# CITlabRostock/citlab-article-separation-new

Hardware: AMD Instinct MI355X
Metric: newspaper pages/sec (ARU-Net seg + GNN relation) at 3000x4500 px (higher is better)
Workload: dtype f32s

## Files before the change

citlab-article-separation-new_amd/csrc/aru_engine.hip:

```cpp
#include <algorithm>
#include <cmath>
#include <cstdlib>
#include <memory>

#include "aru_kernels.h"
#include "res8_kernels.h"
#include "res8v_kernels.h"
#include "bf16_kernels.h"
#include "res8w_kernels.h"
#include "res8ws_kernels.h"
#include "level0_plan.h"
#include "launch_plan.h"
#include "convr_kernels.h"
#include "split_kernels.h"
#include "pyr_kernels.h"
#include "asep_common.h"
#include "aru_pack.h"

using namespace asep;

namespace {

struct Tensor {
    float* p = nullptr;
// ... 26 lines not shown
    asep_aru_cfg cfg{};
    std::map<std::string, PackedConv> convs;
    struct ResB { int C = 0; bf16_t* d_w = nullptr; float* d_b = nullptr; };
    std::map<std::string, ResB> resb;
    std::map<std::string, float*> taps;
    bf16_t* d_r8b_down_w = nullptr;
    float* d_r8b_down_b = nullptr;
    bf16_t* d_r8b_up_w1 = nullptr;
    bf16_t* d_r8f_up_w1 = nullptr;
    bf16_t* d_r8f_down_w1 = nullptr;
    float* d_r8b_down_w1r = nullptr;
    bool use_res32 = true;
    int walk_mode = 1;
    bool use_deconvs = true;
    bool use_convr = true;
    unsigned char* d_zero_trash = nullptr;
    int fused_act = 0;
    bool use_walk = true;
    bf16_t* d_r8b_up_w = nullptr;
    float* d_r8b_up_b = nullptr;
    float* d_r8b_up_b1 = nullptr;
    DirectConv det_first, att_first;
    float* d_r8_down_wr = nullptr;
    float* d_r8_down_br = nullptr;
    float* d_r8_up_w1 = nullptr;
    float* d_r8_up_wr = nullptr;
    float* d_r8_up_br = nullptr;
    float* d_r8_up_b1 = nullptr;
    float* d_r8v_down_wr = nullptr;
    float* d_r8v_up_w1 = nullptr;
    float* d_r8v_up_wr = nullptr;
    bool r8_valu = true;
    bool use_split_walk = true;
    bf16_t* d_r8ws_down_w = nullptr;
    bf16_t* d_r8ws_up_w = nullptr;
    bf16_t* d_r8ws_up_w1 = nullptr;
    bool use_fused8 = true;
    bool fused8_wanted = true;
    bool fused8_var = false;
    float* d_att_head = nullptr;
    bf16_t* d_att_headb = nullptr;
    float* d_logit_w = nullptr;
    float* d_logit_b = nullptr;
    float* d_logit_wd = nullptr;
    float* d_stats = nullptr;
    const float* const* page_stats = nullptr;
    double* d_sums = nullptr;
    struct Lane {
        hipStream_t s = nullptr;
        bool own_stream = false;
        hipStream_t side = nullptr;
        hipEvent_t ev_fork = nullptr, ev_join = nullptr, ev_begin = nullptr, ev_done = nullptr;
        hipStream_t bside = nullptr;
        hipEvent_t ev_bfork = nullptr, ev_bjoin = nullptr;
        BufferPool pool;
        ~Lane() {
            if (ev_fork) (void)hipEventDestroy(ev_fork);
            if (ev_bfork) (void)hipEventDestroy(ev_bfork);
            if (ev_bjoin) (void)hipEventDestroy(ev_bjoin);
            if (ev_join) (void)hipEventDestroy(ev_join);
            if (ev_begin) (void)hipEventDestroy(ev_begin);
            if (ev_done) (void)hipEventDestroy(ev_done);
            if (side) (void)hipStreamDestroy(side);
            if (bside) (void)hipStreamDestroy(bside);
            if (own_stream && s) (void)hipStreamDestroy(s);
        }
// ... 471 lines not shown
    TL out;
    for (const Tensor& t : in) {
        if (kind == POOL_CHANSUM) out.push_back(new_tensor(m, t.H, t.W, 1));
        else out.push_back(new_tensor(m, cdiv(t.H, 2), cdiv(t.W, 2), t.C));
    }
    stream_pass<PoolArgs>(m, in, kind == POOL_MAX ? "maxpool2_kernel" : (kind == POOL_AVG_C1 ? "avgpool2_c1_kernel" : (kind == POOL_AVG_C3 ? "avgpool2_cn_kernel<3>" : "chansum_kernel")), POOL_ITEMS,
        [&](PoolProb& p, size_t i, Chunk& k) {
            k.bytes += tbytes(in[i]) + tbytes(out[i]);
            p.in = in[i].p; p.out = out[i].p; p.H = in[i].H; p.W = in[i].W; p.Ho = out[i].H; p.Wo = out[i].W;
            return kind == POOL_MAX ? out[i].count() / 4 : (size_t)out[i].H * out[i].W;
        }, [&](const PoolArgs& a, dim3 grid) {
            if (kind == POOL_MAX) hipLaunchKernelGGL(maxpool2_kernel, grid, dim3(256), 0, m->stream, a);
            else if (kind == POOL_AVG_C1) hipLaunchKernelGGL(avgpool2_c1_kernel, grid, dim3(256), 0, m->stream, a);
            else if (kind == POOL_AVG_C3) launch_avgpool_c3(m, a, grid);
            else hipLaunchKernelGGL(chansum_kernel, grid, dim3(256), 0, m->stream, a);
        });
    return out;
}

int grid_1d(size_t n) { return (int)std::min<size_t>((n + 255) / 256, 256 * 8); }

std::string res8_what(bool up, const TL& l) {
    return (up ? "unet_up_0 (conv1[16->8]+3xconvR+add) " : "unet_down_0 (conv1+3xconvR+add+pool) ") + dims_of(l);
}

bool r8v_fits(const TL& l) {
    for (const Tensor& t : l)
        if ((size_t)t.H * t.W >= ((size_t)1 << 28)) return false;
    return true;
}

bool r8ws_fits(const Tensor& t) { return walk_region(t.H, t.W).fits; }
bool r8ws_on(asep_aru* m) { return m->split && m->use_split_walk && m->r8_valu && m->cfg.activation == 0 && m->d_r8ws_down_w; }
const int32_t* r8ws_frame_units(asep_aru* m, const Res8Args& a, const std::vector<bool>& walk, int* count) {
    std::string key = "f";
    for (int i = 0; i < a.nprob; ++i) key += ":" + std::to_string(a.p[i].H) + "x" + std::to_string(a.p[i].W) + (walk[i] ? "w" : "t");
    std::vector<int32_t> units;
    for (int i = 0; i < a.nprob; ++i) frame_units(a.p[i].H, a.p[i].W, a.p[i].tiles_x, a.p[i].tile_begin, walk[i], R8_OW, R8_OH * R8_NP, &units);
    *count = (int)units.size();
    auto it = m->sched_cache.find(key);
    if (it != m->sched_cache.end()) return it->second;
    if (units.empty()) return nullptr;
    const int32_t* d = put_table(m, units);
    if (d) m->sched_cache[key] = d;
    return d;
}

void run_res8ws(asep_aru* m, bool up, const Res8Args& a, const std::vector<bool>& walk, const std::string& what) {
    Res8WSArgs wa{};
    int n = 0, items = 0;
    double flops = 0, bytes = 0;
    long strip_rows = 0;
    for (int i = 0; i < a.nprob; ++i) {
        if (!walk[i]) continue;
        const Res8Prob& q = a.p[i];
        Res8WSProb& p = wa.p[n++];
        if (up) { p.skip = q.img; p.dec = q.in1; }
        else { p.img = q.img; p.stats = q.stats; p.pool = q.pool; }
        p.out = q.out;
        p.H = q.H; p.W = q.W;
        const WalkRegion r = walk_region(p.H, p.W);
        p.n_strips = r.n_strips;
        p.y_end = r.y_end;
        strip_rows += (long)r.n_strips * r.rows();
        flops += 2.0 * r.pixels() * (9.0 * (up ? 16 : 1) * 8 + 3 * 9.0 * 64);
        bytes += r.pixels() * ((up ? 64.0 : 4.0) + 32.0 + (p.pool ? 8.0 : 0.0));
    }
    if (!n) return;
    const int band = walk_band(strip_rows, m->num_cus, 4);
    for (int i = 0; i < n; ++i) {
        Res8WSProb& p = wa.p[i];
        p.band = band;
// ... 22 lines not shown
}

void run_res8(asep_aru* m, bool up, const TL& in0, const TL* in1, const std::vector<const float*>& stats, bool want_pool, TL* d_out, TL* pool_out) {
    for (const Tensor& t : in0) {
        d_out->push_back(new_tensor(m, t.H, t.W, 8));
        if (want_pool) pool_out->push_back(new_tensor(m, cdiv(t.H, 2), cdiv(t.W, 2), 8));
    }
    const size_t lds = up ? R8_UP_LDS : R8_DOWN_LDS;
    const char* layer = up ? "unet_up_0" : "unet_down_0";
    for_chunks<Res8Args>(in0.size(), 0.0, [&](Res8Prob& p, size_t i, Chunk& k) {
        k.bytes += tbytes(in0[i]) + (up ? tbytes((*in1)[i]) : 0.0) + tbytes((*d_out)[i]) + (want_pool ? tbytes((*pool_out)[i]) : 0.0);
        p.img = in0[i].p; p.in1 = up ? (*in1)[i].p : nullptr; p.stats = stats.empty() ? nullptr : stats[i];
        p.out = (*d_out)[i].p; p.pool = want_pool ? (*pool_out)[i].p : nullptr;
        p.H = in0[i].H; p.W = in0[i].W;
        set_tiles(p, k.units.next_tiles(p.H, p.W, R8_OW, R8_OH * R8_NP));
        k.flops += 2.0 * in0[i].H * in0[i].W * (9.0 * (up ? 16 : 1) * 8 + 3 * 9.0 * 64);
    }, [&](Res8Args& a, const Chunk& c) {
        const int tiles = c.units.total;
        const double flops = c.flops, bytes = c.bytes;
        const TL sub = c.sub(in0);
        const bool valu = m->r8_valu && r8v_fits(sub);
        if (up) { a.w1 = valu ? m->d_r8v_up_w1 : m->d_r8_up_w1; a.b1 = m->d_r8_up_b1; }
        else { a.w1 = m->det_first.d_w; a.b1 = m->det_first.d_b; }
        a.wr = (const f32x4*)(up ? (valu ? m->d_r8v_up_wr : m->d_r8_up_wr) : (valu ? m->d_r8v_down_wr : m->d_r8_down_wr));
        a.br = up ? m->d_r8_up_br : m->d_r8_down_br;
        const int actv = m->cfg.activation;
        const Res8Kernel k = res8_kernel(up, valu, actv);
        a.sched = tile_schedule(m, a, std::min(tiles, m->num_cus), R8_OH * R8_NP);
        if (valu && r8ws_on(m) && (!up || m->d_r8ws_up_w1)) {
            std::vector<bool> walk(a.nprob);
            bool any = false;
            for (int i = 0; i < a.nprob; ++i) { walk[i] = r8ws_fits(sub[i]); any = any || walk[i]; }
            if (any) {
                int nu = 0;
                Res8Args f = a;
                f.sched = r8ws_frame_units(m, a, walk, &nu);
                if (!f.sched) { set_error("level-0 frame schedule: device allocation failed"); throw ArgError(); }
                f.total_tiles = nu;
                {
                    const double share = (double)nu / tiles;
                    ProfScope ps(m, k.name, flops * share, std::string(layer) + " frame " + dims_of(sub));
                    ps.bytes = bytes * share;
                    hipLaunchKernelGGL(k.fn, dim3(std::min(nu, m->num_cus)), dim3(R8_THREADS), lds, m->stream, f);
                }
                run_res8ws(m, up, a, walk, res8_what(up, sub));
                return;
            }
        }
        ProfScope ps(m, k.name, flops, res8_what(up, sub));
        ps.bytes = bytes;
        if (actv && !valu) { set_error("level-0 block of an elu / leaky graph: image too large for the vector-ALU kernel"); throw ArgError(); }
        hipLaunchKernelGGL(k.fn, dim3(std::min(tiles, m->num_cus)), dim3(R8_THREADS), lds, m->stream, a);
    });
}

void run_res8b_tiles(asep_aru* m, bool up, const TL& a0, const TL* a1, const std::vector<const float*>& stats, bool want_pool, const TL& outs, const TL* pool_out);

void run_res8w(asep_aru* m, bool up, const TL& in0, const TL* dec, const std::vector<const float*>& stats, const TL& outs, const TL* pools) {
    for (size_t c = 0; c < num_chunks(in0.size()); ++c) {
        const size_t b0 = chunk_begin(c), b1 = chunk_end(in0.size(), c);
        Res8WArgs wa{};
        Res8WBArgs ba{};
        double flops = 0, bytes = 0, wshare = 0;
        long strip_rows = 0;
        for (size_t i = b0; i < b1; ++i) {
            Res8WProb& p = wa.p[i - b0];
            if (up) { p.skip = in0[i].bp(); p.dec = (*dec)[i].bp(); }
            else { p.img = in0[i].p; p.stats = stats.empty() ? nullptr : stats[i]; p.pool = pools ? (*pools)[i].bp() : nullptr; }
            p.out = outs[i].bp();
            p.H = in0[i].H; p.W = in0[i].W;
            const WalkRegion r = walk_region(p.H, p.W);
            p.n_strips = r.n_strips;
            p.y_end = r.y_end;
            strip_rows += (long)r.n_strips * r.rows();
            bytes += tbytes(in0[i]) + (up ? tbytes((*dec)[i]) : 0.0) + tbytes(outs[i]) + (pools ? tbytes((*pools)[i]) : 0.0);
            flops += 2.0 * p.H * p.W * (9.0 * (up ? 16 : 1) * 8 + 3 * 9.0 * 64);
            wshare += r.pixels();
        }
// ... 952 lines not shown
    }
    if (cfg->input_pyramid && cfg->compute_dtype == 1) {
        set_error("asep_aru_load: the input-pyramid graph (RU_v2) is served by the fp32 engines (compute_dtype 0 or 2): the bf16 engine's fused block "
                  "tails round conv1's result to bfloat16 before the pooled page's term could be added");
        return nullptr;
    }
    std::map<std::string, HostTensor> blob;
    if (!parse_blob(weight_blob, nbytes, blob)) return nullptr;
    std::map<std::string, std::vector<float>> taps;
    if (cfg->input_pyramid) {
        try {
            blob = split_pyramid_blob(blob, *cfg, taps);
        } catch (const PackRefusal&) {
            return nullptr;
        }
    }
    warn_ignored_switches();
    std::unique_ptr<asep_aru> m(new asep_aru());
    m->cfg = *cfg;
    m->bf16 = cfg->compute_dtype == 1;
    m->split = cfg->compute_dtype == 2;
    if (const char* e = getenv("ASEP_FUSE_POOL")) m->fuse_pool = atoi(e) != 0;
    if (const char* e = getenv("ASEP_FUSE_ACT")) m->fuse_act = atoi(e) != 0;
    if (const char* e = getenv("ASEP_C12")) m->use_c12 = atoi(e) != 0;
    if (const char* e = getenv("ASEP_FUSED8")) m->use_fused8 = atoi(e) != 0;
    m->fused8_wanted = m->use_fused8;
    if (variant) m->use_fused8 = false;
    if (const char* e = getenv("ASEP_R8_VALU")) m->r8_valu = atoi(e) != 0;
    m->fused8_var = variant && !cfg->plain_u && cfg->activation != 0 && m->fused8_wanted && m->r8_valu && m->fuse_act && !m->bf16;
    if (const char* e = getenv("ASEP_XCD_SCHED")) m->use_xcd_sched = atoi(e) != 0;
    if (const char* e = getenv("ASEP_BF_RES32")) m->use_res32 = atoi(e) != 0;
    if (const char* e = getenv("ASEP_BF_CONVR")) m->use_convr = atoi(e) != 0;
    if (const char* e = getenv("ASEP_SPLIT_DECONV")) m->use_deconvs = atoi(e) != 0;
    if (const char* e = getenv("ASEP_SPLIT_WALK")) m->use_split_walk = atoi(e) != 0;
    if (const char* e = getenv("ASEP_BF_WALK")) { m->walk_mode = atoi(e); m->use_walk = m->walk_mode != 0; }
    if (const char* e = getenv("ASEP_LANES")) { m->num_lanes = std::max(1, std::min(4, atoi(e))); m->lanes_forced = true; }
    for (int l = 0; l < m->num_lanes; ++l) {
        std::unique_ptr<asep_aru::Lane> L(new asep_aru::Lane());
        bool ok = hipStreamCreateWithFlags(&L->side, hipStreamNonBlocking) == hipSuccess &&
                  hipStreamCreateWithFlags(&L->bside, hipStreamNonBlocking) == hipSuccess &&
                  hipEventCreateWithFlags(&L->ev_fork, hipEventDisableTiming) == hipSuccess &&
                  hipEventCreateWithFlags(&L->ev_bfork, hipEventDisableTiming) == hipSuccess &&
                  hipEventCreateWithFlags(&L->ev_bjoin, hipEventDisableTiming) == hipSuccess &&
                  hipEventCreateWithFlags(&L->ev_join, hipEventDisableTiming) == hipSuccess &&
                  hipEventCreateWithFlags(&L->ev_begin, hipEventDisableTiming) == hipSuccess &&
                  hipEventCreateWithFlags(&L->ev_done, hipEventDisableTiming) == hipSuccess;
        if (ok && l > 0) { ok = hipStreamCreateWithFlags(&L->s, hipStreamNonBlocking) == hipSuccess; L->own_stream = ok; }
        if (!ok) { set_error("asep_aru_load: cannot create streams/events for lane %d", l); return nullptr; }
        m->lanes.push_back(std::move(L));
    }
    m->cur = m->lanes[0].get();
    for (const auto& t : taps) m->taps[t.first] = m->put(t.second);
    try {
        load_weights(m.get(), blob, variant);
    } catch (const PackRefusal&) {
        return nullptr;
    }
    {
        hipDeviceProp_t prop;
        int dev = 0;
        if (hipGetDevice(&dev) == hipSuccess && hipGetDeviceProperties(&prop, dev) == hipSuccess && prop.multiProcessorCount > 0)
            m->num_cus = prop.multiProcessorCount;
    }
    m->d_stats = m->alloc<float>(2);
    m->d_sums = m->alloc<double>(2);
    m->d_zero_trash = m->alloc<unsigned char>(8192);
    ASEP_HIP_CHECK_THROW(hipMemset(m->d_zero_trash, 0, 8192));
// ... 230 lines not shown
```

citlab-article-separation-new_amd/csrc/level0_plan.h:

```cpp
#pragma once
#include <algorithm>
#include <cstddef>
#include <cstdint>
#include <vector>

namespace asep {

constexpr int R8W_TW = 24;
constexpr int R8W_X0 = 32, R8W_Y0 = 16;

struct WalkRegion {
    int n_strips;
    int y_end;
    int xr;
    bool fits;
    int rows() const { return y_end - R8W_Y0; }
    double pixels() const { return (double)n_strips * R8W_TW * rows(); }
    int bands(int band) const { return (rows() + band - 1) / band; }
    int items(int band) const { return n_strips * bands(band); }
};
inline WalkRegion walk_region(int H, int W) {
    WalkRegion r;
    r.n_strips = (W - 4 - R8W_X0) / R8W_TW;
    r.y_end = R8W_Y0 + 2 * ((H - 4 - R8W_Y0) / 2);
    r.xr = R8W_X0 + R8W_TW * r.n_strips;
    r.fits = r.n_strips >= 4 && H - 4 - R8W_Y0 >= 32 && (size_t)H * W < ((size_t)1 << 28);
    return r;
}

inline int walk_band(long strip_rows, int num_cus, int waves_per_cu) {
    const long slots = (long)waves_per_cu * num_cus;
    const int band = (int)std::min<long>(256, std::max<long>(32, strip_rows / (6 * slots)));
    return (band + 1) & ~1;
}

inline void frame_units(int H, int W, int tiles_x, int tile_begin, bool walk, int unit_w, int unit_h, std::vector<int32_t>* units) {
    const WalkRegion r = walk_region(H, W);
    const int tiles_y = (H + unit_h - 1) / unit_h;
    for (int y = 0; y < tiles_y; ++y)
        for (int x = 0; x < tiles_x; ++x) {
            const int ux0 = x * unit_w, ux1 = std::min(ux0 + unit_w, W), uy0 = y * unit_h, uy1 = std::min(uy0 + unit_h, H);
            const bool frame = !walk || ux0 < R8W_X0 || ux1 > r.xr || uy0 < R8W_Y0 || uy1 > r.y_end;
            if (frame) units->push_back(tile_begin + y * tiles_x + x);
        }
}

struct BorderRect { int x0, y0, x1, y1; };
struct BorderPlan {
    int H, W;
    int nbx;
    int nby;
    int y_end, xr;
    int tiles() const { return 2 * nbx + 2 * nby; }
    BorderRect rect(int t) const {
        int x0, y0, ymax, xmax;
        if (t < nbx) { x0 = 32 * t; y0 = 0; ymax = R8W_Y0; xmax = W; }
        else if (t < 2 * nbx) { x0 = 32 * (t - nbx); y0 = y_end; ymax = H; xmax = W; }
        else if (t < 2 * nbx + nby) { x0 = 0; y0 = R8W_Y0 + 16 * (t - 2 * nbx); ymax = y_end; xmax = R8W_X0; }
        else { x0 = xr; y0 = R8W_Y0 + 16 * (t - 2 * nbx - nby); ymax = y_end; xmax = W; }
        return {x0, y0, std::min(x0 + 32, xmax), std::min(y0 + 16, ymax)};
    }
};
inline BorderPlan border_plan(int H, int W) {
    const WalkRegion r = walk_region(H, W);
    return {H, W, (W + 31) / 32, (r.rows() + 15) / 16, r.y_end, r.xr};
}

}
```

citlab-article-separation-new_amd/csrc/res8_kernels.h:

```cpp
#pragma once
#include "aru_kernels.h"

namespace asep {

#ifdef ASEP_R8_TIMELINE
__device__ unsigned long long r8_tl[16][8][64];
__device__ unsigned long long r8_clk[4];
#define R8_MARK() do { if (blockIdx.x < 16 && lane == 0 && tl_n < 64) r8_tl[blockIdx.x][wave][tl_n++] = clock64(); } while (0)
#else
#define R8_MARK() do { } while (0)
#endif

constexpr int R8_OH = 16, R8_OW = 58;
constexpr int R8_FH = R8_OH + 8;
constexpr int R8_PITCH = 72;
constexpr int R8_IMGP = 76;
constexpr int R8_WAVES = 8;
constexpr int R8_THREADS = R8_WAVES * 64;
#ifndef R8_NP_VALUE
#define R8_NP_VALUE 4
#endif
constexpr int R8_NP = R8_NP_VALUE;

struct Res8Prob {
    const float* img;
    const float* in1;
    const float* stats;
    float* out;
    float* pool;
    int H, W;
    int tiles_x, tile_begin;
};
struct Res8Args {
    Res8Prob p[MAXP];
    int nprob, total_tiles;
    const float* w1;
    const float* b1;
    const f32x4* wr;
    const float* br;
    const int32_t* sched;
};

__device__ __forceinline__ int res8_tile_of(const Res8Args& a, int k) { return a.sched ? a.sched[k] : k; }

__device__ __forceinline__ f32x4 relu4i(f32x4 v) {
    typedef int i32x4 __attribute__((ext_vector_type(4)));
    i32x4 i = __builtin_bit_cast(i32x4, v);
    i.x = max(i.x, 0); i.y = max(i.y, 0); i.z = max(i.z, 0); i.w = max(i.w, 0);
    return __builtin_bit_cast(f32x4, i);
}

__device__ __forceinline__ void r8_load_w(const f32x4* __restrict__ base, int lane, f32x4 (&A)[6]) {
    typedef const f32x4 __attribute__((address_space(1)))* gptr;
    gptr q = (gptr)(base + lane);
    asm volatile("" : "+v"(q));
#pragma unroll
    for (int c = 0; c < 6; ++c) A[c] = q[c * 64];
}

__device__ __forceinline__ int r8_px(int x, int hf) {
#ifdef R8_NO_SWIZZLE
    return x * 8 + hf * 4;
#else
    return ((x >> 1) << 4) + (((((x & 1) << 1) | hf) ^ ((x >> 2) & 3)) << 2);
// ... 440 lines not shown
```

citlab-article-separation-new_amd/csrc/res8v_kernels.h:

```cpp
#pragma once
#include "res8_kernels.h"

namespace asep {

typedef float f32x2 __attribute__((ext_vector_type(2)));
typedef const float __attribute__((address_space(4)))* r8v_cptr;
typedef char __attribute__((address_space(3)))* r8v_lds;

#ifndef R8V_WINO
#define R8V_WINO 0
#endif
#ifndef R8V_WINO_GS
#define R8V_WINO_GS 16
#endif
constexpr int R8V_FILTER = R8V_WINO ? 768 : 576;


__device__ __forceinline__ int r8v_px(int x, int hf) {
    const int P = x >> 1;
    const int g = ((P >> 2) & 1) | ((((P >> 1) ^ (P >> 3)) & 1) << 1);
    return (P << 4) + (((((x & 1) << 1) | hf) ^ g) << 2);
}

template <int ACT>
__device__ __forceinline__ f32x4 r8v_act(f32x4 v) {
    if constexpr (ACT == 0) return relu4i(v);
    else return act4(v, ACT);
}
__device__ __forceinline__ f32x4 r8v_ld(r8v_lds p) { return *reinterpret_cast<const f32x4 __attribute__((address_space(3)))*>(p); }
__device__ __forceinline__ void r8v_st(r8v_lds p, f32x4 v) { *reinterpret_cast<f32x4 __attribute__((address_space(3)))*>(p) = v; }

template <int ODD>
__device__ __forceinline__ void r8v_fma(f32x2& acc, f32x2 pair, f32x2 w) {
    if (ODD) asm("v_pk_fma_f32 %0, %1, %2, %0 op_sel:[1,0,0]" : "+v"(acc) : "v"(pair), "s"(w));
// ... 124 lines not shown
}

template <bool RELU_IN, int ACT = 0>
__device__ __forceinline__ void r8v_conv(const r8v_lds (&a)[4][2], r8v_cptr wl, f32x2 (&acc0)[4], f32x2 (&acc1)[4]) {
    if constexpr (R8V_WINO) r8v_conv_wino<RELU_IN, ACT>(a, wl, acc0, acc1);
    else r8v_conv_direct<RELU_IN, ACT>(a, wl, acc0, acc1);
}

__device__ __forceinline__ f32x4 r8v_lo(const f32x2 (&a)[4]) { return f32x4{a[0].x, a[0].y, a[1].x, a[1].y}; }
__device__ __forceinline__ f32x4 r8v_hi(const f32x2 (&a)[4]) { return f32x4{a[2].x, a[2].y, a[3].x, a[3].y}; }
__device__ __forceinline__ f32x4 r8v_max4(f32x4 a, f32x4 b) { return f32x4{fmaxf(a.x, b.x), fmaxf(a.y, b.y), fmaxf(a.z, b.z), fmaxf(a.w, b.w)}; }
__device__ __forceinline__ f32x4 r8v_upper4(f32x4 v) {
    return f32x4{from_upper_half(v.x), from_upper_half(v.y), from_upper_half(v.z), from_upper_half(v.w)};
}

__device__ __forceinline__ void r8v_pixel_offsets(int tid, int (&poff)[7][2]) {
#pragma unroll
    for (int j = 0; j < 7; ++j) { poff[j][0] = r8v_px(2 * (tid & 31) + j, 0) * 4; poff[j][1] = r8v_px(2 * (tid & 31) + j, 1) * 4; }
}
__device__ __forceinline__ void r8v_window(r8v_lds (&a)[4][2], float* sm, const int (&poff)[7][2], int j0, int row_bytes) {
    asm volatile("" : "+v"(row_bytes));
#pragma unroll
    for (int i = 0; i < 4; ++i)
#pragma unroll
        for (int hf = 0; hf < 2; ++hf) { a[i][hf] = (r8v_lds)reinterpret_cast<char*>(sm) + (poff[j0 + i][hf] + row_bytes); asm volatile("" : "+v"(a[i][hf])); }
}


template <bool RELU_IN, bool FINAL, bool POOL, int ACT = 0>
__device__ __forceinline__ void res8v_stage(float* __restrict__ sm, const float* __restrict__ IN, int in_r0, float* __restrict__ OUT, int out_r0,
                                            int row_start, int nrows, int out_c0, const float* __restrict__ w,
                                            const float* __restrict__ bias, int tid, const int (&poff)[7][2], bool interior,
                                            int fy0, int fx0, int H, int W,
                                            const float* __restrict__ T, int t_r0, float* __restrict__ gout, float* __restrict__ gpool) {
    const int x = out_c0 + 2 * (tid & 31);
    const int gx = fx0 + x;
    const int d_out = FINAL ? 0 : (int)(OUT - IN) * 4 + (in_r0 + 1 - out_r0) * R8_PITCH * 32;
    const int d_t = FINAL ? (int)(T - IN) * 4 + (in_r0 + 1 - t_r0) * R8_PITCH * 32 : 0;
#pragma unroll 1
    for (int r = tid >> 5; r < nrows; r += 16) {
        r8v_cptr wl = (r8v_cptr)w, bl = (r8v_cptr)bias;
        asm volatile("" : "+s"(wl));
        f32x2 acc0[4], acc1[4];
#pragma unroll
        for (int q = 0; q < 4; ++q) { acc0[q] = f32x2{bl[2 * q], bl[2 * q + 1]}; acc1[q] = acc0[q]; }
        const int row = row_start + r;
        r8v_lds a[4][2];
        r8v_window(a, sm, poff, out_c0 - 1, ((int)(IN - sm) + (row - 1 - in_r0) * R8_PITCH * 8) * 4);
        r8v_conv<RELU_IN, ACT>(a, wl, acc0, acc1);
        const int gy = fy0 + row;
        f32x4 p0l = r8v_lo(acc0), p0h = r8v_hi(acc0), p1l = r8v_lo(acc1), p1h = r8v_hi(acc1);
        if (!FINAL) {
            p0l = r8v_act<ACT>(p0l); p0h = r8v_act<ACT>(p0h); p1l = r8v_act<ACT>(p1l); p1h = r8v_act<ACT>(p1h);
            if (!interior) {
                const bool oky = gy >= 0 && gy < H;
                const bool ok0 = oky && gx >= 0 && gx < W, ok1 = oky && gx + 1 >= 0 && gx + 1 < W;
                const f32x4 z = f32x4{0.f, 0.f, 0.f, 0.f};
                p0l = ok0 ? p0l : z; p0h = ok0 ? p0h : z; p1l = ok1 ? p1l : z; p1h = ok1 ? p1h : z;
            }
            r8v_st(a[1][0] + d_out, p0l);
            r8v_st(a[1][1] + d_out, p0h);
            r8v_st(a[2][0] + d_out, p1l);
            r8v_st(a[2][1] + d_out, p1h);
        } else {
            p0l = r8v_act<ACT>(p0l + r8v_ld(a[1][0] + d_t));
            p0h = r8v_act<ACT>(p0h + r8v_ld(a[1][1] + d_t));
            p1l = r8v_act<ACT>(p1l + r8v_ld(a[2][0] + d_t));
            p1h = r8v_act<ACT>(p1h + r8v_ld(a[2][1] + d_t));
            const bool oky = interior || gy < H;
            const bool ok0 = x >= 4 && x < 4 + R8_OW && (interior || gx < W), ok1 = x + 1 >= 4 && x + 1 < 4 + R8_OW && (interior || gx + 1 < W);
            float* o = gout + ((unsigned)gy * (unsigned)W + (unsigned)gx) * 8u;
            if (ok0 && oky) { *reinterpret_cast<f32x4*>(o) = p0l; *reinterpret_cast<f32x4*>(o + 4) = p0h; }
            if (ok1 && oky) { *reinterpret_cast<f32x4*>(o + 8) = p1l; *reinterpret_cast<f32x4*>(o + 12) = p1h; }
            if (POOL && gpool) {
                f32x4 ml = ok1 ? r8v_max4(p0l, p1l) : p0l, mh = ok1 ? r8v_max4(p0h, p1h) : p0h;
                const f32x4 ul = r8v_upper4(ml), uh = r8v_upper4(mh);
                if ((tid & 32) == 0 && ok0 && oky) {
                    if (interior || gy + 1 < H) { ml = r8v_max4(ml, ul); mh = r8v_max4(mh, uh); }
                    const unsigned Wp = (unsigned)(W + 1) >> 1;
                    float* po = gpool + ((unsigned)(gy >> 1) * Wp + (unsigned)(gx >> 1)) * 8u;
                    *reinterpret_cast<f32x4*>(po) = ml;
                    *reinterpret_cast<f32x4*>(po + 4) = mh;
                }
            }
        }
    }
}

template <int ACT = 0>
__global__ __launch_bounds__(R8_THREADS) __attribute__((amdgpu_waves_per_eu(2, 2))) void res8v_down_kernel(const Res8Args a) {
    extern __shared__ __attribute__((aligned(16))) float sm[];
    const float* wr = reinterpret_cast<const float*>(a.wr);
    float* IMG = sm;
    float* T = IMG + R8_FH * R8_IMGP;
    float* R0 = T + 22 * R8_PITCH * 8;
    float* R1 = R0 + 20 * R8_PITCH * 8;
    __shared__ float w1s[9 * 8 + 8];
    const int tid = threadIdx.x;
    if (tid < 72) w1s[tid] = a.w1[tid];
    if (tid < 8) w1s[72 + tid] = a.b1[tid];
    int poff[7][2];
    r8v_pixel_offsets(tid, poff);

    constexpr int NPRE = (R8_FH * R8_IMGP + R8_THREADS - 1) / R8_THREADS;
    float pre[NPRE], pre_mean = 0.f, pre_inv = 1.f;
    unsigned pre_mask = 0;
    auto image_load = [&](int tile_id, int pass) {
        int pi = 0;
        pi = prob_of_tile_search(a, tile_id);
        const Res8Prob& Q = a.p[pi];
        const int t = tile_id - Q.tile_begin;
        const int tyb = t / Q.tiles_x, txb = t - tyb * Q.tiles_x;
        const int qy0 = (tyb * R8_NP + pass) * R8_OH - 4, qx0 = txb * R8_OW - 4;
        pre_mean = 0.f; pre_inv = 1.f; pre_mask = 0;
        if (Q.stats) { pre_mean = Q.stats[0]; pre_inv = Q.stats[1]; }
#pragma unroll
        for (int k = 0; k < NPRE; ++k) {
            const int i = tid + k * R8_THREADS;
            const int r = i / R8_IMGP, c = i - r * R8_IMGP;
            const int gy = qy0 + r, gx = qx0 + c - 2;
            const bool ok = i < R8_FH * R8_IMGP && gy >= 0 && gy < Q.H && gx >= 0 && gx < Q.W;
            pre[k] = Q.img[(size_t)min(max(gy, 0), Q.H - 1) * Q.W + min(max(gx, 0), Q.W - 1)];
            pre_mask |= (ok ? 1u : 0u) << k;
        }
    };
    int tile_id = (int)blockIdx.x < a.total_tiles ? res8_tile_of(a, blockIdx.x) : 0;
    if ((int)blockIdx.x < a.total_tiles) image_load(tile_id, 0);

    for (int k = blockIdx.x; k < a.total_tiles; k += gridDim.x) {
        const bool has_next = k + (int)gridDim.x < a.total_tiles;
        const int next_id = has_next ? res8_tile_of(a, k + gridDim.x) : 0;
        int pi = 0;
        pi = prob_of_tile_search(a, tile_id);
        const Res8Prob& P = a.p[pi];
        const int t = tile_id - P.tile_begin;
        const int tyb = t / P.tiles_x, txb = t - tyb * P.tiles_x;
        const int H = P.H, W = P.W;
        const int fx0 = txb * R8_OW - 4;
#pragma unroll 1
        for (int pass = 0; pass < R8_NP; ++pass) {
            const int fy0 = (tyb * R8_NP + pass) * R8_OH - 4;
            if (fy0 + 4 >= H) break;
            const bool more_passes = pass + 1 < R8_NP && fy0 + 4 + R8_OH < H;
            const bool first = pass == 0;
            const bool interior = fy0 >= 0 && fy0 + R8_FH <= H && fx0 >= 0 && fx0 + R8_PITCH <= W;
            __syncthreads();
            if (!first) {
                constexpr int ROWV = R8_PITCH * 2;
                for (int i = tid; i < 7 * ROWV; i += R8_THREADS) {
                    const int r = i / ROWV, c = i - r * ROWV;
                    f32x4* base = reinterpret_cast<f32x4*>(r < 3 ? T : (r < 5 ? R0 : R1));
                    const int src = r < 3 ? 19 + r : (r < 5 ? 18 + (r - 3) : 16 + (r - 5));
                    const int dst = r < 3 ? 3 + r : (r < 5 ? 2 + (r - 3) : (r - 5));
                    base[dst * ROWV + c] = base[src * ROWV + c];
                }
            }
#pragma unroll
            for (int q = 0; q < NPRE; ++q) {
                const int i = tid + q * R8_THREADS;
                if (i < R8_FH * R8_IMGP) IMG[i] = ((pre_mask >> q) & 1u) ? (pre[q] - pre_mean) * pre_inv : 0.f;
            }
            __syncthreads();
            const int t_lo = first ? 0 : 6 * R8_PITCH;
            for (int i = t_lo + tid; i < 22 * R8_PITCH; i += R8_THREADS) {
                const int r = i / R8_PITCH, c = i - r * R8_PITCH;
                const int gy = fy0 + r + 1, gx = fx0 + c;
                float acc[8];
#pragma unroll
                for (int o = 0; o < 8; ++o) acc[o] = w1s[72 + o];
#pragma unroll
                for (int ky = 0; ky < 3; ++ky)
#pragma unroll
                    for (int kx = 0; kx < 3; ++kx) {
                        const float v = IMG[(r + ky) * R8_IMGP + c + kx + 1];
#pragma unroll
                        for (int o = 0; o < 8; ++o) acc[o] = fmaf(v, w1s[(ky * 3 + kx) * 8 + o], acc[o]);
                    }
                const bool ok = gy >= 0 && gy < H && gx >= 0 && gx < W;
                f32x4 lo = ok ? f32x4{acc[0], acc[1], acc[2], acc[3]} : f32x4{0.f, 0.f, 0.f, 0.f};
                f32x4 hi = ok ? f32x4{acc[4], acc[5], acc[6], acc[7]} : f32x4{0.f, 0.f, 0.f, 0.f};
                *reinterpret_cast<f32x4*>(T + r * R8_PITCH * 8 + r8v_px(c, 0)) = lo;
                *reinterpret_cast<f32x4*>(T + r * R8_PITCH * 8 + r8v_px(c, 1)) = hi;
            }
            __syncthreads();
            res8v_stage<true, false, false, ACT>(sm, T, 1, R0, 2, first ? 2 : 6, first ? 20 : 16, 2, wr, a.br, tid, poff, interior, fy0, fx0, H, W, nullptr, 0, nullptr, nullptr);
            __syncthreads();
            res8v_stage<false, false, false, ACT>(sm, R0, 2, R1, 3, first ? 3 : 5, first ? 18 : 16, 3, wr + R8V_FILTER, a.br + 8, tid, poff, interior, fy0, fx0, H, W, nullptr, 0, nullptr, nullptr);
            __syncthreads();
            if (more_passes) image_load(tile_id, pass + 1);
            else if (has_next) image_load(next_id, 0);
            res8v_stage<false, true, true, ACT>(sm, R1, 3, nullptr, 4, 4, 16, 4, wr + 2 * R8V_FILTER, a.br + 16, tid, poff, interior, fy0, fx0, H, W, T, 1, P.out, P.pool);
        }
        tile_id = next_id;
    }
}

template <int ACT = 0>
__global__ __launch_bounds__(R8_THREADS) __attribute__((amdgpu_waves_per_eu(2, 2))) void res8v_up_kernel(const Res8Args a) {
    extern __shared__ __attribute__((aligned(16))) float sm[];
    const float* wr = reinterpret_cast<const float*>(a.wr);
    float* Pb = sm;
    float* T = Pb + R8_FH * R8_PITCH * 8;
    float* R0 = T + 22 * R8_PITCH * 8;
    float* R1K = R0 + 20 * R8_PITCH * 8;
    char* smb = reinterpret_cast<char*>(sm);
    const int tid = threadIdx.x;
#ifdef ASEP_R8_TIMELINE
    int tl_n = 0;
    const int lane = tid & 63, wave = tid >> 6;
    if (blockIdx.x == 0 && threadIdx.x == 0) { r8_clk[0] = clock64(); r8_clk[1] = wall_clock64(); }
#endif
    int poff[7][2];
    r8v_pixel_offsets(tid, poff);
    constexpr int ROWV = R8_PITCH * 2;
    constexpr int NPF = R8_FH / 3;
    f32x4 pf[NPF];
    const int rg = tid / ROWV, cs = tid - rg * ROWV;
    const int pf_dst = (rg * R8_PITCH * 8 + r8v_px(cs >> 1, cs & 1)) * 4;
    auto tile_load = [&](const float* __restrict__ g, int H_, int W_, int qy0, int qx0, bool carried) {
        const int gx = qx0 + (cs >> 1);
        const bool okc = rg < 3 && gx >= 0 && gx < W_;
        const float* __restrict__ gp = g + ((ptrdiff_t)gx * 8 + (cs & 1) * 4);
#pragma unroll
        for (int k = 0; k < NPF; ++k) {
            const int gy = qy0 + rg + 3 * k;
            f32x4 v = f32x4{0.f, 0.f, 0.f, 0.f};
            if (okc && gy >= 0 && gy < H_ && !(k < 2 && carried)) v = *reinterpret_cast<const f32x4*>(gp + (ptrdiff_t)gy * W_ * 8);
            pf[k] = v;
        }
    };
    auto tile_store = [&](bool carried) {
        if (rg < 3) {
#pragma unroll
            for (int k = 0; k < NPF; ++k) {
                if (k < 2 && carried) continue;
                *reinterpret_cast<f32x4*>(smb + pf_dst + 3 * k * R8_PITCH * 32) = pf[k];
            }
        }
    };
    int tile_id = (int)blockIdx.x < a.total_tiles ? res8_tile_of(a, blockIdx.x) : 0;
    if ((int)blockIdx.x < a.total_tiles) {
        const int first_id = tile_id;
        int qi = 0;
        while (qi + 1 < a.nprob && first_id >= a.p[qi + 1].tile_begin) ++qi;
        const Res8Prob& Q = a.p[qi];
        const int tq = first_id - Q.tile_begin;
        const int qyb = tq / Q.tiles_x, qxb = tq - qyb * Q.tiles_x;
        tile_load(Q.img, Q.H, Q.W, qyb * R8_NP * R8_OH - 4, qxb * R8_OW - 4, false);
    }
    for (int k = blockIdx.x; k < a.total_tiles; k += gridDim.x) {
        const bool has_next = k + (int)gridDim.x < a.total_tiles;
        const int next_id = has_next ? res8_tile_of(a, k + gridDim.x) : 0;
        int pi = 0;
        pi = prob_of_tile_search(a, tile_id);
        const Res8Prob& P = a.p[pi];
        const int t = tile_id - P.tile_begin;
        const int tyb = t / P.tiles_x, txb = t - tyb * P.tiles_x;
        const int H = P.H, W = P.W;
        const int fx0 = txb * R8_OW - 4;
#pragma unroll 1
        for (int pass = 0; pass < R8_NP; ++pass) {
            const int fy0 = (tyb * R8_NP + pass) * R8_OH - 4;
            if (fy0 + 4 >= H) break;
            const bool more_passes = pass + 1 < R8_NP && fy0 + 4 + R8_OH < H;
            const bool first = pass == 0;
            const bool interior = fy0 >= 0 && fy0 + R8_FH <= H && fx0 >= 0 && fx0 + R8_PITCH <= W;
            const int c1_row = first ? 1 : 7, c1_rows = first ? 22 : 16;
            R8_MARK();
            const int r0 = tid >> 5;
            const bool has2 = r0 + 16 < c1_rows;
            r8v_lds wa[4][2];
            r8v_window(wa, sm, poff, 0, (c1_row + r0 - 1) * R8_PITCH * 32);
            f32x2 ta0[4], ta1[4], tb0[4], tb1[4];
            {
                r8v_cptr bl = (r8v_cptr)a.b1;
#pragma unroll
                for (int q = 0; q < 4; ++q) { ta0[q] = f32x2{bl[2 * q], bl[2 * q + 1]}; ta1[q] = ta0[q]; tb0[q] = ta0[q]; tb1[q] = ta0[q]; }
            }
#pragma unroll 1
            for (int half = 0; half < 2; ++half) {
                __syncthreads();
                R8_MARK();
                if (half == 0 && !first) {
                    for (int i = tid; i < 5 * ROWV; i += R8_THREADS) {
                        const int r = i / ROWV, c = i - r * ROWV;
                        f32x4* base = reinterpret_cast<f32x4*>(r < 3 ? T : R0);
                        const int srow = r < 3 ? 19 + r : 18 + (r - 3), drow = r < 3 ? 3 + r : 2 + (r - 3);
                        base[drow * ROWV + c] = base[srow * ROWV + c];
                    }
                }
                tile_store(!first);
                if (half == 0) tile_load(P.in1, H, W, fy0, fx0, !first);
                __syncthreads();
                R8_MARK();
                r8v_cptr wl = (r8v_cptr)(a.w1 + half * R8V_FILTER);
                asm volatile("" : "+s"(wl));
                r8v_conv<false>(wa, wl, ta0, ta1);
                if (has2) {
// ... 35 lines not shown
                    r8v_st(wa[1][1] + D2, v0h);
                    r8v_st(wa[2][0] + D2, v1l);
                    r8v_st(wa[2][1] + D2, v1h);
                }
            }
            R8_MARK();
            __syncthreads();
            R8_MARK();
            res8v_stage<true, false, false, ACT>(sm, T, 1, R0, 2, first ? 2 : 6, first ? 20 : 16, 2, wr, a.br, tid, poff, interior, fy0, fx0, H, W, nullptr, 0, nullptr, nullptr);
            R8_MARK();
            __syncthreads();
            R8_MARK();
            res8v_stage<false, false, false, ACT>(sm, R0, 2, Pb, 3, first ? 3 : 5, first ? 18 : 16, 3, wr + R8V_FILTER, a.br + 8, tid, poff, interior, fy0, fx0, H, W, nullptr, 0, nullptr, nullptr);
            if (!first) {
                for (int i = tid; i < 2 * ROWV; i += R8_THREADS)
                    reinterpret_cast<f32x4*>(Pb)[i] = reinterpret_cast<const f32x4*>(R1K)[i];
            }
            R8_MARK();
            __syncthreads();
            R8_MARK();
            if (more_passes) {
                for (int i = tid; i < 2 * ROWV; i += R8_THREADS)
                    reinterpret_cast<f32x4*>(R1K)[i] = reinterpret_cast<const f32x4*>(Pb)[16 * ROWV + i];
            }
            if (more_passes || has_next) {
                const float* g = P.img;
                int H_ = H, W_ = W, qy0 = fy0 + R8_OH, qx0 = fx0;
                if (!more_passes) {
                    int qi = 0;
                    while (qi + 1 < a.nprob && next_id >= a.p[qi + 1].tile_begin) ++qi;
                    const Res8Prob& Q = a.p[qi];
                    const int tq = next_id - Q.tile_begin;
                    const int qyb = tq / Q.tiles_x, qxb = tq - qyb * Q.tiles_x;
                    g = Q.img; H_ = Q.H; W_ = Q.W; qy0 = qyb * R8_NP * R8_OH - 4; qx0 = qxb * R8_OW - 4;
                }
                tile_load(g, H_, W_, qy0, qx0, more_passes);
            }
            R8_MARK();
            res8v_stage<false, true, false, ACT>(sm, Pb, 3, nullptr, 4, 4, 16, 4, wr + 2 * R8V_FILTER, a.br + 16, tid, poff, interior, fy0, fx0, H, W, T, 1, P.out, nullptr);
            R8_MARK();
        }
        tile_id = next_id;
    }
#ifdef ASEP_R8_TIMELINE
    if (blockIdx.x == 0 && threadIdx.x == 0) { r8_clk[2] = clock64(); r8_clk[3] = wall_clock64(); }
#endif
}

template <bool OUTBF = false>
__global__ __launch_bounds__(256) void att_headv_kernel(const AttHeadArgs a) {
    constexpr int LH = ATT_TH + 3, LW = ATT_TW + 4;
    __shared__ __attribute__((aligned(16))) float img[LH * LW];
    const int tid = threadIdx.x;
    int pi = 0;
    pi = prob_of_tile(a, (int)blockIdx.x);
    const C1Prob& P = a.p[pi];
    const int tile = blockIdx.x - P.tile_begin;
    const int ty = tile / P.tiles_x, tx = tile - ty * P.tiles_x;
    const int x0 = tx * ATT_TW, y0 = ty * ATT_TH;
    const int H = P.H, W = P.W;
    float mean = 0.f, inv = 1.f;
    if (P.stats) { mean = P.stats[0]; inv = P.stats[1]; }
    {
        constexpr int NSL = (LH * LW + 255) / 256;
        float st[NSL];
#pragma unroll
        for (int k = 0; k < NSL; ++k) {
            const int i = min(tid + k * 256, LH * LW - 1);
            const int r = i / LW, c = i - r * LW;
            st[k] = P.img[(size_t)min(max(y0 - 1 + r, 0), H - 1) * W + min(max(x0 - 1 + c, 0), W - 1)];
        }
#pragma unroll
        for (int k = 0; k < NSL; ++k) {
            const int i = tid + k * 256;
            if (i >= LH * LW) break;
// ... 257 lines not shown
```

Measured before the change: 151.5.

## Clip level-0 frame kernel to border passes and overlap it with walker on side stream

The frame schedule for the level-0 residual block now encodes per-unit pass ranges, so the vector-ALU kernel runs only the passes that touch the border frame rather than full multi-pass units. It also suppresses output stores inside the walker rectangle, and sorts entries by cost. When a side stream is available, the frame kernel runs concurrently with the split-walk kernel, ordered by fork/join events. This removes redundant interior work the walker already covers, at the cost of extra scheduling logic, an odd-size guard, and possible contention between the two concurrent kernels.

```diff
diff --git a/citlab-article-separation-new_amd/csrc/aru_engine.hip b/citlab-article-separation-new_amd/csrc/aru_engine.hip
--- a/citlab-article-separation-new_amd/csrc/aru_engine.hip
+++ b/citlab-article-separation-new_amd/csrc/aru_engine.hip
@@ -82,6 +82,7 @@
     float* d_r8v_up_wr = nullptr;
     bool r8_valu = true;
     bool use_split_walk = true;
+    bool frame_clip = true;
     bf16_t* d_r8ws_down_w = nullptr;
     bf16_t* d_r8ws_up_w = nullptr;
     bf16_t* d_r8ws_up_w1 = nullptr;
@@ -619,12 +620,18 @@
 
 bool r8ws_fits(const Tensor& t) { return walk_region(t.H, t.W).fits; }
 bool r8ws_on(asep_aru* m) { return m->split && m->use_split_walk && m->r8_valu && m->cfg.activation == 0 && m->d_r8ws_down_w; }
-const int32_t* r8ws_frame_units(asep_aru* m, const Res8Args& a, const std::vector<bool>& walk, int* count) {
-    std::string key = "f";
+const int32_t* r8ws_frame_units(asep_aru* m, const Res8Args& a, const std::vector<bool>& walk, bool clip, int* count, int* entries) {
+    std::string key = clip ? "fc" : "f";
     for (int i = 0; i < a.nprob; ++i) key += ":" + std::to_string(a.p[i].H) + "x" + std::to_string(a.p[i].W) + (walk[i] ? "w" : "t");
     std::vector<int32_t> units;
     for (int i = 0; i < a.nprob; ++i) frame_units(a.p[i].H, a.p[i].W, a.p[i].tiles_x, a.p[i].tile_begin, walk[i], R8_OW, R8_OH * R8_NP, &units);
     *count = (int)units.size();
+    if (clip) {
+        units.clear();
+        for (int i = 0; i < a.nprob; ++i) frame_entries(a.p[i].H, a.p[i].W, a.p[i].tiles_x, a.p[i].tile_begin, walk[i], R8_OW, R8_OH, R8_NP, &units);
+        frame_cost_order(&units, R8_NP);
+    }
+    *entries = (int)units.size();
     auto it = m->sched_cache.find(key);
     if (it != m->sched_cache.end()) return it->second;
     if (units.empty()) return nullptr;
@@ -713,18 +720,39 @@
             bool any = false;
             for (int i = 0; i < a.nprob; ++i) { walk[i] = r8ws_fits(sub[i]); any = any || walk[i]; }
             if (any) {
-                int nu = 0;
+                const bool clip = m->frame_clip && tiles < (1 << FRAME_UNIT_BITS);
+                int nu = 0, ne = 0;
                 Res8Args f = a;
-                f.sched = r8ws_frame_units(m, a, walk, &nu);
+                f.sched = r8ws_frame_units(m, a, walk, clip, &nu, &ne);
                 if (!f.sched) { set_error("level-0 frame schedule: device allocation failed"); throw ArgError(); }
-                f.total_tiles = nu;
+                f.total_tiles = ne;
+                for (int i = 0; clip && i < a.nprob; ++i) {
+                    const FrameClip c = frame_clip(a.p[i].H, a.p[i].W, walk[i]);
+                    if ((c.x1 | c.y1 | R8W_X0 | R8W_Y0) & 1) { set_error("level-0 frame clip: odd walker rectangle"); throw ArgError(); }
+                    f.p[i].clip_x1 = c.x1; f.p[i].clip_y1 = c.y1;
+                }
+                asep_aru::Lane& L = *m->cur;
+                const bool beside = clip && !m->profiling && L.bside;
+                bool frame_first = !beside;
+#ifdef ASEP_ABLATION
+                if (const char* e = getenv("ASEP_FRAME_FIRST")) frame_first = atoi(e) != 0 || !beside;
+#endif
+                if (beside) {
+                    ASEP_HIP_CHECK_THROW(hipEventRecord(L.ev_bfork, m->stream));
+                    ASEP_HIP_CHECK_THROW(hipStreamWaitEvent(L.bside, L.ev_bfork, 0));
+                }
+                if (!frame_first) run_res8ws(m, up, a, walk, res8_what(up, sub));
                 {
                     const double share = (double)nu / tiles;
                     ProfScope ps(m, k.name, flops * share, std::string(layer) + " frame " + dims_of(sub));
                     ps.bytes = bytes * share;
-                    hipLaunchKernelGGL(k.fn, dim3(std::min(nu, m->num_cus)), dim3(R8_THREADS), lds, m->stream, f);
+                    hipLaunchKernelGGL(k.fn, dim3(std::min(ne, m->num_cus)), dim3(R8_THREADS), lds, beside ? L.bside : m->stream, f);
                 }
-                run_res8ws(m, up, a, walk, res8_what(up, sub));
+                if (frame_first) run_res8ws(m, up, a, walk, res8_what(up, sub));
+                if (beside) {
+                    ASEP_HIP_CHECK_THROW(hipEventRecord(L.ev_bjoin, L.bside));
+                    ASEP_HIP_CHECK_THROW(hipStreamWaitEvent(m->stream, L.ev_bjoin, 0));
+                }
                 return;
             }
         }
@@ -1743,7 +1771,7 @@
     if (const char* e = getenv("ASEP_BF_RES32")) m->use_res32 = atoi(e) != 0;
     if (const char* e = getenv("ASEP_BF_CONVR")) m->use_convr = atoi(e) != 0;
     if (const char* e = getenv("ASEP_SPLIT_DECONV")) m->use_deconvs = atoi(e) != 0;
-    if (const char* e = getenv("ASEP_SPLIT_WALK")) m->use_split_walk = atoi(e) != 0;
+    if (const char* e = getenv("ASEP_SPLIT_WALK")) { m->use_split_walk = atoi(e) != 0; m->frame_clip = atoi(e) != 2; }
     if (const char* e = getenv("ASEP_BF_WALK")) { m->walk_mode = atoi(e); m->use_walk = m->walk_mode != 0; }
     if (const char* e = getenv("ASEP_LANES")) { m->num_lanes = std::max(1, std::min(4, atoi(e))); m->lanes_forced = true; }
     for (int l = 0; l < m->num_lanes; ++l) {
diff --git a/citlab-article-separation-new_amd/csrc/level0_plan.h b/citlab-article-separation-new_amd/csrc/level0_plan.h
--- a/citlab-article-separation-new_amd/csrc/level0_plan.h
+++ b/citlab-article-separation-new_amd/csrc/level0_plan.h
@@ -45,6 +45,43 @@
         }
 }
 
+constexpr int FRAME_UNIT_BITS = 24;
+constexpr int32_t frame_entry(int unit, int p0, int p1, int np) { return (int32_t)(unit | p0 << FRAME_UNIT_BITS | (np - p1) << (FRAME_UNIT_BITS + 4)); }
+constexpr int frame_entry_unit(int32_t e) { return e & ((1 << FRAME_UNIT_BITS) - 1); }
+constexpr int frame_entry_p0(int32_t e) { return (e >> FRAME_UNIT_BITS) & 7; }
+constexpr int frame_entry_p1(int32_t e, int np) { return np - ((e >> (FRAME_UNIT_BITS + 4)) & 7); }
+
+struct FrameClip { int x1, y1; };
+inline FrameClip frame_clip(int H, int W, bool walk) {
+    const WalkRegion r = walk_region(H, W);
+    return walk ? FrameClip{r.xr, r.y_end} : FrameClip{0, 0};
+}
+
+inline void frame_entries(int H, int W, int tiles_x, int tile_begin, bool walk, int unit_w, int pass_h, int np, std::vector<int32_t>* entries) {
+    std::vector<int32_t> units;
+    frame_units(H, W, tiles_x, tile_begin, walk, unit_w, pass_h * np, &units);
+    if (!walk) { entries->insert(entries->end(), units.begin(), units.end()); return; }
+    const WalkRegion r = walk_region(H, W);
+    for (const int32_t u : units) {
+        const int t = u - tile_begin, x = t % tiles_x, y = t / tiles_x;
+        const int ux0 = x * unit_w, ux1 = std::min(ux0 + unit_w, W);
+        const bool side = ux0 < R8W_X0 || ux1 > r.xr;
+        int p0 = -1;
+        for (int p = 0; p <= np; ++p) {
+            const int py0 = (y * np + p) * pass_h, py1 = std::min(py0 + pass_h, H);
+            const bool frame = p < np && py0 < H && (side || py0 < R8W_Y0 || py1 > r.y_end);
+            if (frame && p0 < 0) p0 = p;
+            if (!frame && p0 >= 0) { entries->push_back(frame_entry(u, p0, p, np)); p0 = -1; }
+        }
+    }
+}
+
+inline void frame_cost_order(std::vector<int32_t>* entries, int np) {
+    std::stable_sort(entries->begin(), entries->end(), [np](int32_t a, int32_t b) {
+        return frame_entry_p1(a, np) - frame_entry_p0(a) > frame_entry_p1(b, np) - frame_entry_p0(b);
+    });
+}
+
 struct BorderRect { int x0, y0, x1, y1; };
 struct BorderPlan {
     int H, W;
diff --git a/citlab-article-separation-new_amd/csrc/res8_kernels.h b/citlab-article-separation-new_amd/csrc/res8_kernels.h
--- a/citlab-article-separation-new_amd/csrc/res8_kernels.h
+++ b/citlab-article-separation-new_amd/csrc/res8_kernels.h
@@ -30,6 +30,7 @@
     float* pool;
     int H, W;
     int tiles_x, tile_begin;
+    int clip_x1, clip_y1;
 };
 struct Res8Args {
     Res8Prob p[MAXP];
diff --git a/citlab-article-separation-new_amd/csrc/res8v_kernels.h b/citlab-article-separation-new_amd/csrc/res8v_kernels.h
--- a/citlab-article-separation-new_amd/csrc/res8v_kernels.h
+++ b/citlab-article-separation-new_amd/csrc/res8v_kernels.h
@@ -1,5 +1,6 @@
 #pragma once
 #include "res8_kernels.h"
+#include "level0_plan.h"
 
 namespace asep {
 
@@ -190,7 +191,7 @@
                                             int row_start, int nrows, int out_c0, const float* __restrict__ w,
                                             const float* __restrict__ bias, int tid, const int (&poff)[7][2], bool interior,
                                             int fy0, int fx0, int H, int W,
-                                            const float* __restrict__ T, int t_r0, float* __restrict__ gout, float* __restrict__ gpool) {
+                                            const float* __restrict__ T, int t_r0, float* __restrict__ gout, float* __restrict__ gpool, int keep = 1) {
     const int x = out_c0 + 2 * (tid & 31);
     const int gx = fx0 + x;
     const int d_out = FINAL ? 0 : (int)(OUT - IN) * 4 + (in_r0 + 1 - out_r0) * R8_PITCH * 32;
@@ -225,7 +226,7 @@
             p0h = r8v_act<ACT>(p0h + r8v_ld(a[1][1] + d_t));
             p1l = r8v_act<ACT>(p1l + r8v_ld(a[2][0] + d_t));
             p1h = r8v_act<ACT>(p1h + r8v_ld(a[2][1] + d_t));
-            const bool oky = interior || gy < H;
+            const bool oky = keep && (interior || gy < H);
             const bool ok0 = x >= 4 && x < 4 + R8_OW && (interior || gx < W), ok1 = x + 1 >= 4 && x + 1 < 4 + R8_OW && (interior || gx + 1 < W);
             float* o = gout + ((unsigned)gy * (unsigned)W + (unsigned)gx) * 8u;
             if (ok0 && oky) { *reinterpret_cast<f32x4*>(o) = p0l; *reinterpret_cast<f32x4*>(o + 4) = p0h; }
@@ -245,6 +246,15 @@
     }
 }
 
+static_assert(R8_NP <= 7, "a schedule entry has three bits for a pass number");
+__device__ __forceinline__ int res8v_entry_of(const Res8Args& a, int k) { return a.sched ? a.sched[k] : k; }
+__device__ __forceinline__ int r8v_keep(const Res8Prob& P, int fy0, int fx0, int tid) {
+    const int gy = fy0 + 4 + (tid >> 5), gx = fx0 + 4 + 2 * (tid & 31);
+    int keep = (gx >= R8W_X0 && gx < P.clip_x1 && gy >= R8W_Y0 && gy < P.clip_y1) ? 0 : 1;
+    asm volatile("" : "+v"(keep));
+    return keep;
+}
+
 template <int ACT = 0>
 __global__ __launch_bounds__(R8_THREADS) __attribute__((amdgpu_waves_per_eu(2, 2))) void res8v_down_kernel(const Res8Args a) {
     extern __shared__ __attribute__((aligned(16))) float sm[];
@@ -282,12 +292,13 @@
             pre_mask |= (ok ? 1u : 0u) << k;
         }
     };
-    int tile_id = (int)blockIdx.x < a.total_tiles ? res8_tile_of(a, blockIdx.x) : 0;
-    if ((int)blockIdx.x < a.total_tiles) image_load(tile_id, 0);
+    int entry = (int)blockIdx.x < a.total_tiles ? res8v_entry_of(a, blockIdx.x) : 0;
+    if ((int)blockIdx.x < a.total_tiles) image_load(frame_entry_unit(entry), frame_entry_p0(entry));
 
     for (int k = blockIdx.x; k < a.total_tiles; k += gridDim.x) {
         const bool has_next = k + (int)gridDim.x < a.total_tiles;
-        const int next_id = has_next ? res8_tile_of(a, k + gridDim.x) : 0;
+        const int next_entry = has_next ? res8v_entry_of(a, k + gridDim.x) : 0;
+        const int tile_id = frame_entry_unit(entry), p0 = frame_entry_p0(entry), p1 = frame_entry_p1(entry, R8_NP);
         int pi = 0;
         pi = prob_of_tile_search(a, tile_id);
         const Res8Prob& P = a.p[pi];
@@ -296,11 +307,11 @@
         const int H = P.H, W = P.W;
         const int fx0 = txb * R8_OW - 4;
 #pragma unroll 1
-        for (int pass = 0; pass < R8_NP; ++pass) {
+        for (int pass = p0; pass < p1; ++pass) {
             const int fy0 = (tyb * R8_NP + pass) * R8_OH - 4;
             if (fy0 + 4 >= H) break;
-            const bool more_passes = pass + 1 < R8_NP && fy0 + 4 + R8_OH < H;
-            const bool first = pass == 0;
+            const bool more_passes = pass + 1 < p1 && fy0 + 4 + R8_OH < H;
+            const bool first = pass == p0;
             const bool interior = fy0 >= 0 && fy0 + R8_FH <= H && fx0 >= 0 && fx0 + R8_PITCH <= W;
             __syncthreads();
             if (!first) {
@@ -346,10 +357,11 @@
             res8v_stage<false, false, false, ACT>(sm, R0, 2, R1, 3, first ? 3 : 5, first ? 18 : 16, 3, wr + R8V_FILTER, a.br + 8, tid, poff, interior, fy0, fx0, H, W, nullptr, 0, nullptr, nullptr);
             __syncthreads();
             if (more_passes) image_load(tile_id, pass + 1);
-            else if (has_next) image_load(next_id, 0);
-            res8v_stage<false, true, true, ACT>(sm, R1, 3, nullptr, 4, 4, 16, 4, wr + 2 * R8V_FILTER, a.br + 16, tid, poff, interior, fy0, fx0, H, W, T, 1, P.out, P.pool);
-        }
-        tile_id = next_id;
+            else if (has_next) image_load(frame_entry_unit(next_entry), frame_entry_p0(next_entry));
+            res8v_stage<false, true, true, ACT>(sm, R1, 3, nullptr, 4, 4, 16, 4, wr + 2 * R8V_FILTER, a.br + 16, tid, poff, interior, fy0, fx0, H, W, T, 1, P.out, P.pool,
+                                                r8v_keep(P, fy0, fx0, tid));
+        }
+        entry = next_entry;
     }
 }
 
@@ -396,19 +408,20 @@
             }
         }
     };
-    int tile_id = (int)blockIdx.x < a.total_tiles ? res8_tile_of(a, blockIdx.x) : 0;
+    int entry = (int)blockIdx.x < a.total_tiles ? res8v_entry_of(a, blockIdx.x) : 0;
     if ((int)blockIdx.x < a.total_tiles) {
-        const int first_id = tile_id;
+        const int first_id = frame_entry_unit(entry);
         int qi = 0;
         while (qi + 1 < a.nprob && first_id >= a.p[qi + 1].tile_begin) ++qi;
         const Res8Prob& Q = a.p[qi];
         const int tq = first_id - Q.tile_begin;
         const int qyb = tq / Q.tiles_x, qxb = tq - qyb * Q.tiles_x;
-        tile_load(Q.img, Q.H, Q.W, qyb * R8_NP * R8_OH - 4, qxb * R8_OW - 4, false);
+        tile_load(Q.img, Q.H, Q.W, (qyb * R8_NP + frame_entry_p0(entry)) * R8_OH - 4, qxb * R8_OW - 4, false);
     }
     for (int k = blockIdx.x; k < a.total_tiles; k += gridDim.x) {
         const bool has_next = k + (int)gridDim.x < a.total_tiles;
-        const int next_id = has_next ? res8_tile_of(a, k + gridDim.x) : 0;
+        const int next_entry = has_next ? res8v_entry_of(a, k + gridDim.x) : 0;
+        const int tile_id = frame_entry_unit(entry), next_id = frame_entry_unit(next_entry), p0 = frame_entry_p0(entry), p1 = frame_entry_p1(entry, R8_NP);
         int pi = 0;
         pi = prob_of_tile_search(a, tile_id);
         const Res8Prob& P = a.p[pi];
@@ -417,11 +430,11 @@
         const int H = P.H, W = P.W;
         const int fx0 = txb * R8_OW - 4;
 #pragma unroll 1
-        for (int pass = 0; pass < R8_NP; ++pass) {
+        for (int pass = p0; pass < p1; ++pass) {
             const int fy0 = (tyb * R8_NP + pass) * R8_OH - 4;
             if (fy0 + 4 >= H) break;
-            const bool more_passes = pass + 1 < R8_NP && fy0 + 4 + R8_OH < H;
-            const bool first = pass == 0;
+            const bool more_passes = pass + 1 < p1 && fy0 + 4 + R8_OH < H;
+            const bool first = pass == p0;
             const bool interior = fy0 >= 0 && fy0 + R8_FH <= H && fx0 >= 0 && fx0 + R8_PITCH <= W;
             const int c1_row = first ? 1 : 7, c1_rows = first ? 22 : 16;
             R8_MARK();
@@ -523,15 +536,16 @@
                     const Res8Prob& Q = a.p[qi];
                     const int tq = next_id - Q.tile_begin;
                     const int qyb = tq / Q.tiles_x, qxb = tq - qyb * Q.tiles_x;
-                    g = Q.img; H_ = Q.H; W_ = Q.W; qy0 = qyb * R8_NP * R8_OH - 4; qx0 = qxb * R8_OW - 4;
+                    g = Q.img; H_ = Q.H; W_ = Q.W; qy0 = (qyb * R8_NP + frame_entry_p0(next_entry)) * R8_OH - 4; qx0 = qxb * R8_OW - 4;
                 }
                 tile_load(g, H_, W_, qy0, qx0, more_passes);
             }
             R8_MARK();
-            res8v_stage<false, true, false, ACT>(sm, Pb, 3, nullptr, 4, 4, 16, 4, wr + 2 * R8V_FILTER, a.br + 16, tid, poff, interior, fy0, fx0, H, W, T, 1, P.out, nullptr);
+            res8v_stage<false, true, false, ACT>(sm, Pb, 3, nullptr, 4, 4, 16, 4, wr + 2 * R8V_FILTER, a.br + 16, tid, poff, interior, fy0, fx0, H, W, T, 1, P.out, nullptr,
+                                                 r8v_keep(P, fy0, fx0, tid));
             R8_MARK();
         }
-        tile_id = next_id;
+        entry = next_entry;
     }
 #ifdef ASEP_R8_TIMELINE
     if (blockIdx.x == 0 && threadIdx.x == 0) { r8_clk[2] = clock64(); r8_clk[3] = wall_clock64(); }
```

New measurement: 152.2 (median of 6 runs). Within noise of the previous version (+0.4%).
